# EmbersArc/EiCOS

Measured on NVIDIA B200. Metric: SOCP solves/sec, higher is better.
Workload: dtype f64

## Files before the change

### eicos_b200/csrc/engine.cu

```cuda
#include "engine.hpp"
#include "backend.hpp"
#include "tile_program.hpp"

#include <algorithm>
#include <cstdint>
#ifdef EICOS_EMU
#include <thread>
#endif

namespace eicos
{

#ifndef EICOS_EMU
#define EI_DEFINE_KERNEL(name, fn, minblocks) EI_DEFINE_KERNEL_(name, fn, EI_MAX_THREADS, minblocks, 0)
#define EI_DEFINE_KERNEL1(name, fn) EI_DEFINE_KERNEL_(name, fn, 32, 8, 0)
#define EI_DEFINE_KERNEL_(name, fn, maxthreads, minblocks, JOBS)                                           \
    __global__ void __launch_bounds__(maxthreads, minblocks) name(const __grid_constant__ KArgs a) \
    {                                                                                          \
        extern __shared__ double smem[];                                                       \
        Team tm;                                                                               \
        tm.pl = threadIdx.x & 31;                                                              \
        tm.lane = tm.pl * VEC;                                                                 \
        tm.wk = threadIdx.x >> 5;                                                              \
        tm.nwk = blockDim.x >> 5;                                                              \
// ... 58 lines not shown
                fn(tm_, (args), tile_);                                                           \
            };                                                                                    \
            std::vector<std::thread> th_;                                                         \
            for (int wk_ = 1; wk_ < nw_; wk_++)                                                   \
                th_.emplace_back(body_, wk_);                                                     \
            body_(0);                                                                             \
            for (auto &t_ : th_)                                                                  \
                t_.join();                                                                        \
        }                                                                                         \
    } while (0)
#endif

#ifdef EICOS_EMU
static void eicos_compact_emu(const KArgs &a, const MoveRanges &mr, const int *moves, int nmoves)
{
    for (int q = 0; q < nmoves; q++)
    {
        compact_move(a, mr, moves[2 * q], moves[2 * q + 1], 0, 1);
        compact_vacate(a, moves[2 * q]);
    }
}
#endif

constexpr int MAX_SW_SLOTS = 16, MAX_FA_SLOTS = 24;

int Engine::tile_width() { return TILE; }

bool Engine::pair_solves(int) const { return force_pair_ > 0; }

bool Engine::deep_ring(int ctas) const
{
    if (force_variant_ >= 0)
        return force_variant_ > 0;
    long long per_sm = (long long)((size_t)227 * 1024 / (smem_prog_[M_VARIANTS - 1] + 1024));
    if (const char *v = std::getenv("EICOS_DEEP_CTAS_PER_SM"))
        per_sm = std::atoi(v);
    return (long long)ctas <= per_sm * sms_;
}

bool Engine::wide_launch(int ctas) const
{
    if (force_wide_ >= 0)
        return force_wide_ > 0;
    const long long per_sm = (long long)((size_t)227 * 1024 / (smem_wide_ + 1024));
    return per_sm > 0 && (long long)ctas <= per_sm * sms_;
}

namespace
{
template <class T>
T *upload(const std::vector<T> &v, std::vector<void *> &owned, be::stream_t s)
{
    T *d = (T *)be::alloc(v.size() * sizeof(T));
    be::h2d(d, v.data(), v.size() * sizeof(T), s);
    owned.push_back(d);
    return d;
}
inline be::stream_t S_(void *p) { return (be::stream_t)(intptr_t)p; }

dvec expanded_geq(const Symbolic &S)
{
    dvec g(S.mt, 1.0);
    for (int i = 0; i < S.m; i++)
        g[S.zk[i]] = S.Geq[i];
    return g;
}
}

void Engine::build_layout(const Symbolic &S, bool acc_rows)
{
    int at = 0;
    auto take = [&](int rows) {
        const int o = at;
        at += rows;
        return o;
    };
    Layout &L = L_;
    L.chb = take(S.N);
    L.w = take(S.N);
    L.s = take(S.mt);
    L.lam = take(S.mt);
    L.wb = take(S.N);
    L.bs = take(S.mt);
    L.blam = take(S.mt);
    L.r = take(S.N);
    L.lpv = take(S.l);
    L.lpw = take(S.l);
    L.cpar = take(S.nc * CP_COUNT);
    L.cq = take(S.qtot);
    L.V = take((int)S.Vslot.size());
    L.Lx = take(S.nnzL);
    L.D = take(S.N);
    L.Dinv = take(S.N);
    L.rhs1 = take(S.N);
    L.rhs2 = take(S.N);
    L.sol1 = take(S.N);
    L.sol2 = take(S.N);
    L.xw = take(S.N);
    L.dxr = take(S.N);
    L.e = take(S.N);
    L.xw2 = take(S.N);
    L.dxr2 = take(S.N);
    L.e2 = take(S.N);
    L.dsw = take(S.mt);
    L.wdz = take(S.mt);
    L.dsaff = take(S.mt);
    L.ds1 = take(S.mt);
    L.Gx = take(pim_ ? S.G.nnz() : 0);
    L.Ax = take(pim_ ? S.A.nnz() : 0);
    L.eq = take(pim_ ? S.N : 0);
    L.sc = take(S_COUNT);
    L.acc = acc_rows ? take(S.nnzL) : -1;
    L.rows_total = at;
    L.irows_total = J_COUNT;
}

void Engine::upload_pattern(const Symbolic &S)
{
    be::stream_t st = S_(stream_);
    int sw_budget = MAX_SW_SLOTS, fa_budget = MAX_FA_SLOTS;
    if (const char *v = std::getenv("EICOS_MAX_SW_SLOTS"))
        sw_budget = std::max(1, std::min(MAX_SW_SLOTS, std::atoi(v)));
    if (const char *v = std::getenv("EICOS_MAX_FA_SLOTS"))
        fa_budget = std::max(1, std::min(MAX_FA_SLOTS, std::atoi(v)));
    try
    {
        build_streams(S, L_, workers_, sw_budget, fa_budget, H_, pim_);
    }
    catch (const MachineOutOfSlots &)
    {
        if (L_.acc >= 0)
            throw;
        build_layout(S, true);
        build_streams(S, L_, workers_, sw_budget, fa_budget, H_, pim_);
    }
    Lp_ = S.Lp;
    DevPattern &P = P_;
    P.n = S.n;
    P.p = S.p;
    P.m = S.m;
    P.l = S.l;
    P.nc = S.nc;
    P.N = S.N;
    P.mt = S.mt;
    P.qtot = S.qtot;
    P.nnzL = S.nnzL;
    P.nnzV = (int)S.Vslot.size();
    P.maxcol = S.maxcol;
    P.pim = pim_ ? 1 : 0;
    P.nnzG = S.G.nnz();
    P.nnzA = S.A.nnz();
    if (pim_)
    {
        P.Gp = upload(S.G.p, owned_, st);
        P.Gi = upload(S.G.i, owned_, st);
        P.Ap = upload(S.A.p, owned_, st);
        P.Ai = upload(S.A.i, owned_, st);
        P.Grp = upload(S.Gr.p, owned_, st);
        P.Grv = upload(S.Gr.v, owned_, st);
        P.Arp = upload(S.Ar.p, owned_, st);
        P.Arv = upload(S.Ar.v, owned_, st);
        P.cone_z = upload(S.cone_z, owned_, st);
    }
    P.cone_dim = upload(S.q, owned_, st);
    P.cone_k = upload(S.cone_k, owned_, st);
    P.cone_q = upload(S.cone_q, owned_, st);
    P.zk = upload(S.zk, owned_, st);
// ... 410 lines not shown
            a.initialize = init;
            pick(2 * tiles);
            if (pair_solves(tiles))
            {
                a.njobs = 1;
                EI_TIMED(1, EI_LAUNCH(eicos_solve_kkt_pair, tile_solve_kkt<2>, tiles, threads1, smem_pair_, st, a));
            }
            else if (wide_launch(2 * tiles))
            {
                a.variant = force_variant_ == 0 ? 0 : M_VARIANTS - 1;
                EI_TIMED(1, EI_LAUNCH_JOBS(eicos_solve_kkt_wide, tile_solve_kkt<1>, tiles, 2, threads_wide, smem_wide_, st, a));
            }
            else
                EI_TIMED(1, EI_LAUNCH_JOBS(eicos_solve_kkt, tile_solve_kkt<1>, tiles, 2, threads1, smem_prog_[a.variant], st, a));
            stt.solve_launches++;
            stt.solve_launch_tiles += (long long)tiles * 2;
        };
        auto kkt_rhs2 = [&](int nitrow) {
            a.job[0] = {L_.rhs2, L_.sol2, nitrow, 1};
            a.njobs = 1;
            a.initialize = 0;
            pick(tiles);
            if (wide_launch(tiles))
            {
                a.variant = force_variant_ == 0 ? 0 : M_VARIANTS - 1;
                EI_TIMED(1, EI_LAUNCH_JOBS(eicos_solve_kkt_wide, tile_solve_kkt<1>, tiles, 1, threads_wide, smem_wide_, st, a));
            }
            else
                EI_TIMED(1, EI_LAUNCH_JOBS(eicos_solve_kkt, tile_solve_kkt<1>, tiles, 1, threads1, smem_prog_[a.variant], st, a));
            stt.solve_launches++;
            stt.solve_launch_tiles += tiles;
        };

        EI_TIMED(2, EI_LAUNCH(eicos_load_inputs, tile_load, tiles, threads, smem_common_, st, a));
        if (pim_)
            EI_TIMED(2, EI_LAUNCH(eicos_equilibrate, tile_equil, tiles, threads, smem_common_, st, a));
        EI_TIMED(2, EI_LAUNCH(eicos_init, tile_init, tiles, threads, smem_common_, st, a));
        factor();
        kkt_pair(1, J_NIT1, J_NIT2);
        EI_TIMED(2, EI_LAUNCH(eicos_init_point, tile_init_point, tiles, threads, smem_common_, st, a));

        for (int it = 0; it <= iter_max_ + 1; it++)
        {
            be::zero(active_count_, sizeof(unsigned int), st);
            if (wide_launch(tiles))
                EI_TIMED(3, EI_LAUNCH(eicos_residuals_wide, tile_resid, tiles, threads_wide, smem_wide_, st, a));
            else
                EI_TIMED(3, EI_LAUNCH(eicos_residuals, tile_resid, tiles, threads1, smem_resid_, st, a));
            EI_TIMED(4, EI_LAUNCH(eicos_iter_head, tile_head, tiles, threads, smem_common_, st, a));
            stt.resid_launches++, stt.vector_launches++;
            stt.resid_launch_tiles += tiles, stt.vector_launch_tiles += tiles;
            stt.ipm_iterations++;
            be::d2h(host_pinned_, active_count_, sizeof(unsigned int), st);
            be::sync(st);
            const long long nactive = host_pinned_[0];
            if (nactive == 0)
                break;
            if (compaction_ && !keep_sticky && tiles >= 8 && nactive * 4 <= (long long)tiles * TILE * 3)
            {
                EI_TIMED(2, EI_LAUNCH(eicos_store_outputs, tile_store, tiles, threads, smem_common_, st, a));
                be::d2h_2d(status_host_, TILE * sizeof(int), iws_ + (size_t)J_STATUS * TILE,
                           (size_t)L_.irows_total * TILE * sizeof(int), TILE * sizeof(int), tiles, st);
                be::sync(st);
                const int new_tiles = (int)((nactive + TILE - 1) / TILE);
                int nmoves = 0, hole = 0;
                const int keep = new_tiles * TILE;
                for (int src = keep; src < tiles * TILE; src++)
                {
                    if (status_host_[src] != ST_ACTIVE)
                        continue;
                    while (hole < keep && status_host_[hole] == ST_ACTIVE)
                        hole++;
                    if (hole >= keep)
                        throw std::logic_error("compaction: no free slot");
                    moves_host_[2 * nmoves] = src;
                    moves_host_[2 * nmoves + 1] = hole++;
                    nmoves++;
                }
                if (nmoves > 0)
                {
                    be::h2d(moves_dev_, moves_host_, 2 * (size_t)nmoves * sizeof(int), st);
                    MoveRanges mr;
                    const int rr[14] = {L_.chb, P_.N,
                                        L_.w, (L_.blam + P_.mt) - L_.w,
                                        L_.r, P_.N,
                                        L_.lpv, (L_.V + P_.nnzV) - L_.lpv,
                                        L_.rhs1, 2 * P_.N,
                                        L_.sc, S_COUNT,
                                        L_.Gx, L_.sc - L_.Gx};
                    mr.n = 7;
                    for (int k = 0; k < 14; k++)
                        mr.r[k] = rr[k];
#ifndef EICOS_EMU
                    eicos_compact<<<nmoves, 128, 0, st>>>(a, mr, moves_dev_);
#else
                    eicos_compact_emu(a, mr, moves_dev_, nmoves);
#endif
                    stt.launches++;
                    stt.compactions++;
                }
                tiles = new_tiles;
            }
            factor();
            kkt_pair(0, -1, -1);
            EI_TIMED(4, EI_LAUNCH(eicos_iter_mid, tile_mid, tiles, threads, smem_common_, st, a));
            kkt_rhs2(J_NIT3);
            EI_TIMED(4, EI_LAUNCH(eicos_iter_tail, tile_tail, tiles, threads, smem_common_, st, a));
            stt.vector_launches += 2;
            stt.vector_launch_tiles += 2 * (long long)tiles;
        }
        EI_TIMED(2, EI_LAUNCH(eicos_store_outputs, tile_store, tiles, threads, smem_common_, st, a));
    }
    be::d2h(host_pinned_ + 2, ir_rounds_, 8 * sizeof(unsigned long long), st);
#ifndef EICOS_EMU
    if (timing)
    {
        ev_end = ev();
        EI_CUDA(cudaEventRecord(ev_end, st));
    }
    EI_CUDA(cudaGetLastError());
#endif
    be::sync(st);
    std::memcpy(&stt.ir_rounds, host_pinned_ + 2, sizeof(unsigned long long));
    std::memcpy(&stt.lane_rounds, host_pinned_ + 2 + 2 * 6, sizeof(unsigned long long));
    std::memcpy(stt.kkt_phase_cycles, host_pinned_ + 4, 5 * sizeof(unsigned long long));
#ifndef EICOS_EMU
    if (timing)
    {
        float ms = 0;
        EI_CUDA(cudaEventElapsedTime(&ms, ev_begin, ev_end));
        stt.ms_total = ms;
        for (const Span &sp : spans)
        {
            EI_CUDA(cudaEventElapsedTime(&ms, sp.a, sp.b));
            (sp.cls == 0 ? stt.ms_factor : sp.cls == 1 ? stt.ms_solve : stt.ms_other) += ms;
            if (sp.cls == 3)
                stt.ms_resid += ms;
            if (sp.cls == 4)
                stt.ms_vector += ms;
        }
    }
#endif
#undef EI_TIMED
}

void Engine::debug_factor_init(int batch, const double *d_c, const double *d_h, const double *d_b,
                               const double *base_c, const double *base_h, const double *base_b,
                               double *h_Lx, double *h_D, double *h_sol1, double *h_sol2, int *h_nit)
{
    be::set_device(device_);
    be::stream_t st = S_(stream_);
    if (batch > cap_tiles_ * TILE)
        throw std::invalid_argument("debug_factor_init: batch exceeds workspace capacity");
    KArgs a;
    std::memset(&a, 0, sizeof(a));
    a.P = P_;
    a.L = L_;
    a.ws = ws_;
    a.iws = iws_;
    a.in_c = d_c;
    a.in_h = d_h;
    a.in_b = d_b;
    a.base_c = base_vec_;
    a.base_h = base_vec_ + P_.n;
    a.base_b = base_vec_ + P_.n + P_.m;
    if (base_c)
        be::h2d(base_vec_, base_c, P_.n * sizeof(double), st);
// ... 70 lines not shown
```

### eicos_b200/csrc/layout.hpp

```cpp
#pragma once

#include <cstddef>

namespace eicos
{

enum : int
{
    ST_ACTIVE = -1000,
    EXIT_OPTIMAL = 0,
    EXIT_PINF = 1,
    EXIT_DINF = 2,
    EXIT_MAXIT = -1,
    EXIT_NUMERICS = -2,
    EXIT_OUTCONE = -3,
    EXIT_FATAL = -7,
    EXIT_INACC = 10,
    EXIT_NOT_CONVERGED = -87
};

enum ScalarRow : int
{
    S_KAP, S_TAU, S_CX, S_BY, S_HZ,
    S_PCOST, S_DCOST, S_PRES, S_DRES, S_PINFRES, S_DINFRES, S_GAP, S_RELGAP,
    S_SIGMA, S_MU, S_STEP, S_STEP_AFF, S_KAPOVERT,
    S_WORK_END,
    S_BEST = S_WORK_END,
    S_BEST_END = S_BEST + S_WORK_END,
    S_RT = S_BEST_END, S_NX, S_NY, S_NZ, S_NS, S_HRESX, S_HRESY, S_HRESZ,
    S_RESX0, S_RESY0, S_RESZ0, S_PRES_PREV,
    S_DTAU_DENOM, S_DTAUAFF, S_DKAPAFF,
    S_RHSMAX1, S_RHSMAX2,
    S_RED,
    S_COUNT = S_RED + 14
};

enum IntRow : int
{
    J_ITER, J_PINF, J_DINF, J_HAS_PINFRES, J_HAS_DINFRES, J_HAS_RELGAP, J_NIT1, J_NIT2, J_NIT3,
    J_WORK_END,
    J_BEST = J_WORK_END,
    J_BEST_END = J_BEST + J_WORK_END,
    J_STATUS = J_BEST_END,
    J_INST,
    J_STORED,
    J_COUNT
};

struct Layout
{
    int chb;
    int w;
    int s, lam;
    int wb, bs, blam;
    int r;
    int lpv, lpw;
    int cpar, cq;
    int V;
    int Lx, D, Dinv;
    int rhs1, rhs2, sol1, sol2;
    int xw, dxr, e;
    int xw2, dxr2, e2;
    int dsw, wdz, dsaff, ds1;
    int Gx, Ax, eq;
    int sc;
    int acc;
    int rows_total;
    int irows_total;
};

struct DevMachine
{
    const int *ops;
    int nchunks;
    int nld_chunks;
    int ring_groups;
    int ring_row0;
};

enum ConeParam : int
{
    CP_ETA, CP_ETA2, CP_A, CP_D1, CP_U0, CP_U1, CP_V1, CP_W, CP_COUNT
};

struct DevPattern
{
    int n, p, m, l, nc, N, mt, qtot, nnzL, nnzV, maxcol;
    const int *cone_dim, *cone_k, *cone_q;
    const int *zk;
    const double *xeq, *Aeq, *GeqE;
    DevMachine fw[2], bw[2], bwp[2], mv[2];
    const int *fw_ld[2][2][2], *bw_ld[2][2][2], *mv_ld[2][2];
    DevMachine rs[4], mvw[4];
    const int *rs_ld[4], *mvw_ld[2][4];
    DevMachine fw2, bw2, bwp2, mv2;
    const int *fw2_ld[2], *bw2_ld[2], *mv2_ld;
    int mv_rows;
    int sw_budget, fa_budget, pair_budget;
    DevMachine fa[2];
    const int *fa_ld[2];
    int pim, nnzG, nnzA;
    const int *Gp, *Gi, *Ap, *Ai, *Grp, *Grv, *Arp, *Arv, *cone_z;
    const int *Vkind;
};

}
```

### eicos_b200/csrc/tile_program.hpp

```cpp
#pragma once

#include "layout.hpp"
#include "streams.hpp"
#include "symbolic.hpp"

#include <cfloat>
#include <cmath>

#ifdef EICOS_EMU
#include <barrier>
#define EI_DEV inline
#define EI_LDG(p) (*(p))
#define EI_CLOCK() 0ll
#else
#include <cuda_runtime.h>
#define EI_DEV __device__ __forceinline__
#define EI_LDG(p) __ldg(p)
#define EI_CLOCK() clock64()
#endif

#ifndef EICOS_VEC
#define EICOS_VEC 2
#endif

namespace eicos
{

#ifdef EICOS_EMU
constexpr int LANES = 1;
#else
constexpr int LANES = 32;
#endif
constexpr int VEC = EICOS_VEC;
constexpr int TILE = LANES * VEC;
constexpr int KRED = 7;

struct alignas(VEC >= 2 ? 16 : 8) vd
{
    double v[VEC];
};
struct vb
{
    bool v[VEC];
};
#define VFOR for (int c_ = 0; c_ < VEC; c_++)

EI_DEV vd vset(double s)
{
    vd r;
    VFOR r.v[c_] = s;
    return r;
}
EI_DEV vd operator+(vd a, vd b) { VFOR a.v[c_] += b.v[c_]; return a; }
EI_DEV vd operator-(vd a, vd b) { VFOR a.v[c_] -= b.v[c_]; return a; }
EI_DEV vd operator*(vd a, vd b) { VFOR a.v[c_] *= b.v[c_]; return a; }
EI_DEV vd operator/(vd a, vd b) { VFOR a.v[c_] /= b.v[c_]; return a; }
EI_DEV vd operator-(vd a) { VFOR a.v[c_] = -a.v[c_]; return a; }
EI_DEV vd operator+(vd a, double b) { VFOR a.v[c_] += b; return a; }
EI_DEV vd operator-(vd a, double b) { VFOR a.v[c_] -= b; return a; }
EI_DEV vd operator+(double b, vd a) { VFOR a.v[c_] = b + a.v[c_]; return a; }
EI_DEV vd operator-(double b, vd a) { VFOR a.v[c_] = b - a.v[c_]; return a; }
EI_DEV vd operator*(vd a, double b) { VFOR a.v[c_] *= b; return a; }
EI_DEV vd operator*(double b, vd a) { VFOR a.v[c_] = b * a.v[c_]; return a; }
EI_DEV vd operator/(vd a, double b) { VFOR a.v[c_] /= b; return a; }
EI_DEV vd operator/(double b, vd a) { VFOR a.v[c_] = b / a.v[c_]; return a; }
EI_DEV vd &operator+=(vd &a, vd b) { VFOR a.v[c_] += b.v[c_]; return a; }
EI_DEV vd &operator-=(vd &a, vd b) { VFOR a.v[c_] -= b.v[c_]; return a; }
EI_DEV vd vfnma(vd v, vd a, vd b)
{
    VFOR v.v[c_] = fma(-a.v[c_], b.v[c_], v.v[c_]);
    return v;
}
EI_DEV vd vfnma(vd v, double a, vd b)
{
    VFOR v.v[c_] = fma(-a, b.v[c_], v.v[c_]);
    return v;
}
EI_DEV vd vsqrt(vd a) { VFOR a.v[c_] = sqrt(a.v[c_]); return a; }
EI_DEV vd vabs(vd a) { VFOR a.v[c_] = fabs(a.v[c_]); return a; }
EI_DEV bool ei_isnan(double v) { return v != v; }
EI_DEV double dmax(double a, double b) { return a > b ? a : b; }
EI_DEV double dmin(double a, double b) { return b < a ? b : a; }
EI_DEV vd vmax(vd a, vd b) { VFOR a.v[c_] = dmax(a.v[c_], b.v[c_]); return a; }
EI_DEV vd vmin(vd a, vd b) { VFOR a.v[c_] = dmin(a.v[c_], b.v[c_]); return a; }
EI_DEV vd vsel(vb m, vd a, vd b) { VFOR a.v[c_] = m.v[c_] ? a.v[c_] : b.v[c_]; return a; }
EI_DEV vb vbset(bool s)
{
    vb r;
    VFOR r.v[c_] = s;
    return r;
}
EI_DEV vb operator&&(vb a, vb b) { VFOR a.v[c_] = a.v[c_] && b.v[c_]; return a; }
EI_DEV vb operator||(vb a, vb b) { VFOR a.v[c_] = a.v[c_] || b.v[c_]; return a; }
EI_DEV vb operator!(vb a) { VFOR a.v[c_] = !a.v[c_]; return a; }
EI_DEV bool vany(vb a)
{
    bool r = false;
    VFOR r = r || a.v[c_];
    return r;
}
EI_DEV bool vall(vb a)
{
    bool r = true;
    VFOR r = r && a.v[c_];
    return r;
}

EI_DEV vd vload(const double *p) { return *reinterpret_cast<const vd *>(p); }
EI_DEV void vstore(double *p, vd v) { *reinterpret_cast<vd *>(p) = v; }

#ifdef EICOS_EMU
struct i4
{
    int x, y, z, w;
};
EI_DEV i4 ldg4(const int *p) { return i4{p[0], p[1], p[2], p[3]}; }
#else
typedef int4 i4;
EI_DEV i4 ldg4(const int *p) { return __ldg(reinterpret_cast<const int4 *>(p)); }
#endif
struct alignas(16) d2
{
    double x, y;
};
EI_DEV d2 ldg2(const double *p)
{
#ifdef EICOS_EMU
    return d2{p[0], p[1]};
#else
    const double2 v = __ldg(reinterpret_cast<const double2 *>(p));
    return d2{v.x, v.y};
#endif
}

struct RowRef
{
    double *p;
    EI_DEV operator vd() const { return vload(p); }
    EI_DEV void operator=(vd v) const { vstore(p, v); }
    EI_DEV void operator=(double s) const { vstore(p, vset(s)); }
    EI_DEV void operator+=(vd v) const { vstore(p, vload(p) + v); }
    EI_DEV void operator-=(vd v) const { vstore(p, vload(p) - v); }
    EI_DEV void operator*=(double s) const { vstore(p, vload(p) * s); }
    EI_DEV void operator*=(vd s) const { vstore(p, vload(p) * s); }
    EI_DEV void operator=(const RowRef &o) const { vstore(p, vload(o.p)); }
};
#define ROWD(base, r) (RowRef{(base) + (size_t)(r) * TILE})
#define ROWC(base, r, c) ((base)[(size_t)(r) * TILE + (c)])

struct KArgs
{
    DevPattern P;
    Layout L;
    double *ws;
    int *iws;
    int batch;
    int first;
    const double *in_c, *in_h, *in_b;
    const double *base_c, *base_h, *base_b;
// ... 1440 lines not shown
        const vd res = resv[0], b = bv[0], own = ownv[0];
        if (kind == RS_PRE_X)
            r[RS_HX2] += res * res;
        else if (kind == RS_PRE_Y)
            r[RS_HY2] += res * res;
        else if (kind == RS_PRE_Z)
            r[RS_HZ2] += res * res;
        else
        {
            if (kind == RS_FIN_X)
            {
                r[RS_RX2] += res * res;
                r[RS_CX] += b * own;
                r[RS_NX2] += own * own;
            }
            else if (kind == RS_FIN_Y)
            {
                r[RS_RY2] += res * res;
                r[RS_BY] += b * own;
                r[RS_NY2] += own * own;
            }
            else if (kind == RS_FIN_Z)
            {
                r[RS_RZ2] += res * res;
                r[RS_HZ] += b * own;
                r[RS_NZ2] += own * own;
            }
            else
            {
                r[RS_NS2] += res * res;
                r[RS_GAP] += res * own;
                if (kind == RS_FIRST_PRE_Z)
                    r[RS_HZ2] += res * res;
            }
        }
    }
};

EI_DEV void tile_resid(const Team &tm, const KArgs &a, int tile)
{
    const TileMem t = tile_mem(tm, a, tile);
    const vb act = lane_active(tm, t);
    if (!tm.any(act))
        return;
    const DevPattern &P = a.P;
    const Layout &L = a.L;
    double *T = t.T;
    const bool wide = tm.nwk >= M_MV_PARTS;
    vd tot[RS_NRED];
    for (int k = 0; k < RS_NRED; k++)
        tot[k] = vset(0.0);
    const auto run_part = [&](int part, double *mem) {
        ResidFin fin;
        for (int k = 0; k < RS_NRED; k++)
            fin.r[k] = vset(0.0);
        Machine mm;
        mm.init(tm, mem);
        MRun r;
        r.prog = P.rs[part];
        r.ld = P.rs_ld[part];
        r.Tb = t.Tb;
        r.out = r.out2 = r.outB = r.out2B = T + (size_t)L.r * TILE;
        r.a_one = false;
        mm.run<MC_CONST | MC_POS | MC_BKEEP | MC_FIN | MC_X3, 1>(tm, r, fin);
        for (int k = 0; k < RS_NRED; k++)
            tot[k] = part == 0 || wide ? fin.r[k] : tot[k] + fin.r[k];
    };
    if (P.mv_rows > 0)
    {
        if (wide)
        {
            if (tm.wk < M_MV_PARTS)
                run_part(tm.wk, tm.pbuf + (size_t)tm.wk * a.part_doubles);
            team_sum<RS_NRED>(tm, tot);
        }
        else if (tm.wk == 0)
            for (int part = 0; part < M_MV_PARTS; part++)
                run_part(part, tm.pbuf);
    }
    if (tm.wk == 0)
        for (int k = 0; k < RS_NRED; k++)
            ROWD(T, L.sc + S_RED + k) = tot[k];
}

EI_DEV void tile_head(const Team &tm, const KArgs &a, int tile)
{
    const TileMem t = tile_mem(tm, a, tile);
    const vb act = lane_active(tm, t);
    if (!tm.any(act))
        return;
    const DevPattern &P = a.P;
    const Layout &L = a.L;
    double *T = t.T;
    int *I = t.I;
    const int n = P.n, p = P.p, zb = P.n + P.p;
    const vd tau = ROWD(T, L.sc + S_TAU), kap = ROWD(T, L.sc + S_KAP);
    enum { HX2, RX2, CX, NX2, HY2, RY2, BY, NY2, HZ2, RZ2, HZ, NZ2, NS2, GAP, NRED };
    static_assert(NRED == 14, "S_RED holds 14 rows");
    vd r[NRED];
    for (int k = 0; k < NRED; k++)
        r[k] = ROWD(T, L.sc + S_RED + k);

    vb restore = vbset(false), save = vbset(false), fin = vbset(false), cont = vbset(false);
    vd ftau = tau;
    WState wsv[VEC], bsv[VEC];
    double rtv[VEC], ppv[VEC];
    int codev[VEC];
    VFOR
    {
        const int c = c_;
        WState &w = wsv[c], &best = bsv[c];
        ws_load(tm, T, I, L.sc, 0, 0, c, w);
        ws_load(tm, T, I, L.sc, S_BEST, J_BEST, c, best);
        const double tau_c = tau.v[c], kap_c = kap.v[c];
        const double hresx = sqrt(r[HX2].v[c]), hresy = sqrt(r[HY2].v[c]), hresz = sqrt(r[HZ2].v[c]);
        const double nx = sqrt(r[NX2].v[c]), ny = sqrt(r[NY2].v[c]), nz = sqrt(r[NZ2].v[c]), ns = sqrt(r[NS2].v[c]);
        const double cx = r[CX].v[c], by = p > 0 ? r[BY].v[c] : 0., hz = r[HZ].v[c];
        const double rt = kap_c + cx + by + hz;
        w.d[S_CX] = cx;
        w.d[S_BY] = by;
        w.d[S_HZ] = hz;
        w.d[S_GAP] = r[GAP].v[c];
        w.d[S_MU] = (r[GAP].v[c] + kap_c * tau_c) / ((P.l + P.nc) + 1);
        w.d[S_KAPOVERT] = kap_c / tau_c;
        w.d[S_PCOST] = cx / tau_c;
        w.d[S_DCOST] = -(hz + by) / tau_c;
        if (w.d[S_PCOST] < 0.)
        {
            w.i[J_HAS_RELGAP] = 1;
            w.d[S_RELGAP] = w.d[S_GAP] / (-w.d[S_PCOST]);
        }
        else if (w.d[S_DCOST] > 0.)
        {
            w.i[J_HAS_RELGAP] = 1;
            w.d[S_RELGAP] = w.d[S_GAP] / w.d[S_DCOST];
        }
        else
            w.i[J_HAS_RELGAP] = 0;
        const double resx0 = ROWC(T, L.sc + S_RESX0, c), resy0 = ROWC(T, L.sc + S_RESY0, c), resz0 = ROWC(T, L.sc + S_RESZ0, c);
        const double nry = p > 0 ? sqrt(r[RY2].v[c]) / dmax(resy0 + nx, 1.) : 0.;
        const double nrz = sqrt(r[RZ2].v[c]) / dmax(resz0 + nx + ns, 1.);
        w.d[S_PRES] = dmax(nry, nrz) / tau_c;
        w.d[S_DRES] = sqrt(r[RX2].v[c]) / dmax(resx0 + ny + nz, 1.) / tau_c;
        if ((hz + by) / dmax(ny + nz, 1.) < -Settings::reltol)
        {
            w.i[J_HAS_PINFRES] = 1;
            w.d[S_PINFRES] = hresx / dmax(ny + nz, 1.);
        }
        if (cx / dmax(nx, 1.) < -Settings::reltol)
        {
            w.i[J_HAS_DINFRES] = 1;
            w.d[S_DINFRES] = dmax(hresy / dmax(nx, 1.), hresz / dmax(nx + ns, 1.));
        }

        const int iter = w.i[J_ITER];
        double pres_prev = ROWC(T, L.sc + S_PRES_PREV, c);
        int code = ST_ACTIVE;
        bool rst = false, sav = false;
        if (act.v[c])
        {
            if (iter > 0 && (w.d[S_PRES] > Settings::safeguard * pres_prev || w.d[S_GAP] < 0.))
            {
                rst = true;
                w = best;
                code = ws_check_exit(w, true);
                if (code == EXIT_NOT_CONVERGED)
                    code = EXIT_NUMERICS;
            }
            else
            {
                pres_prev = w.d[S_PRES];
                code = ws_check_exit(w, false);
                if (code == EXIT_NOT_CONVERGED)
                {
                    if (iter > 0 && w.d[S_STEP] == Settings::stepmin * Settings::gamma)
                    {
                        rst = true;
                        w = best;
                        code = ws_check_exit(w, true);
                        if (code == EXIT_NOT_CONVERGED)
                            code = EXIT_NUMERICS;
                    }
                    else if (iter == a.iter_max)
                    {
                        if (!ws_better(w, best))
                        {
                            rst = true;
                            w = best;
                        }
                        code = ws_check_exit(w, true);
                        if (code == EXIT_NOT_CONVERGED)
                            code = EXIT_MAXIT;
                    }
                    else if (ei_isnan(w.d[S_PCOST]))
                    {
                        if (!(iter == 0 || ws_better(w, best)))
                        {
                            rst = true;
                            w = best;
                            code = ws_check_exit(w, true);
                            if (code == EXIT_NOT_CONVERGED)
                                code = EXIT_NUMERICS;
                        }
                    }
                    else
                        code = ST_ACTIVE;
                }
            }
            if (code == ST_ACTIVE && (iter == 0 || ws_better(w, best)))
            {
                sav = true;
                best = w;
            }
        }
        restore.v[c] = rst;
        save.v[c] = sav;
        fin.v[c] = act.v[c] && code != ST_ACTIVE;
        cont.v[c] = act.v[c] && code == ST_ACTIVE;
        ftau.v[c] = w.d[S_TAU];
        rtv[c] = rt;
        ppv[c] = pres_prev;
        codev[c] = code;
    }
    tm.sync();
    if (tm.wk == 0)
        VFOR if (act.v[c_])
        {
            ws_store(tm, T, I, L.sc, 0, 0, c_, wsv[c_]);
            if (save.v[c_])
                ws_store(tm, T, I, L.sc, S_BEST, J_BEST, c_, bsv[c_]);
            ROWC(T, L.sc + S_RT, c_) = rtv[c_];
            ROWC(T, L.sc + S_PRES_PREV, c_) = ppv[c_];
            ROWC(I, J_STATUS, c_) = codev[c_];
        }

    if (!tm.any(restore || fin) && tm.all(save || !act))
    {
        const int ins[1] = {L.w};
        ew_rows<1, 8>(tm, T, P.N, ins, [&](int q, const vd *x) { ROWD(T, L.wb + q) = x[0]; });
        const int inz[2] = {L.s, L.lam};
        ew_rows<2, 6>(tm, T, P.mt, inz, [&](int e, const vd *x) {
            ROWD(T, L.bs + e) = x[0];
            ROWD(T, L.blam + e) = x[1];
        });
    }
    else if (tm.any(restore || save || fin))
    {
        const bool any_fin = tm.any(fin);
        {
            const int ins[2] = {L.w, L.wb};
            ew_rows<2, 6>(tm, T, P.N, ins, [&](int q, const vd *x) {
                vd v = vsel(restore, x[1], x[0]);
                ROWD(T, L.wb + q) = vsel(save, v, x[1]);
                if (any_fin && P.pim)
                    v = vsel(fin, v / (vd(ROWD(T, L.eq + q)) * ftau), v);
                else if (any_fin)
                {
                    const double eq = q < n ? EI_LDG(P.xeq + q) : (q < zb ? EI_LDG(P.Aeq + q - n) : EI_LDG(P.GeqE + q - zb));
                    v = vsel(fin, v / (eq * ftau), v);
                }
                ROWD(T, L.w + q) = v;
            });
        }
        {
            const int ins[4] = {L.s, L.lam, L.bs, L.blam};
            ew_rows<4, 3>(tm, T, P.mt, ins, [&](int e, const vd *x) {
                vd sv = vsel(restore, x[2], x[0]), lv = vsel(restore, x[3], x[1]);
                ROWD(T, L.bs + e) = vsel(save, sv, x[2]);
                ROWD(T, L.blam + e) = vsel(save, lv, x[3]);
                if (any_fin && P.pim)
                    sv = vsel(fin, sv * (vd(ROWD(T, L.eq + zb + e)) / ftau), sv);
                else if (any_fin)
                    sv = vsel(fin, sv * (EI_LDG(P.GeqE + e) / ftau), sv);
                ROWD(T, L.s + e) = sv;
                ROWD(T, L.lam + e) = lv;
            });
        }
    }
    if (!tm.any(cont))
        return;
    tm.sync();
#ifndef EICOS_EMU
    if (tm.wk == 0 && a.active_count)
    {
        int mine = 0;
        VFOR mine += cont.v[c_] ? 1 : 0;
        for (int o = 16; o > 0; o >>= 1)
            mine += __shfl_xor_sync(0xffffffffu, mine, o);
        if (tm.pl == 0)
            atomicAdd(a.active_count, (unsigned)mine);
    }
#else
    if (tm.wk == 0 && a.active_count)
        VFOR if (cont.v[c_]) *a.active_count += 1;
#endif

    const int sz = L.w + zb;
    const bool lp_only = P.nc == 0;
    if (lp_only && tm.all(cont))
    {
        const int ins[2] = {L.s, sz};
        ew_rows<2, 6>(tm, T, P.l, ins, [&](int k, const vd *x) {
            const vd v = x[0] / x[1];
            const vd w = vsqrt(v);
            ROWD(T, L.lpv + k) = -v;
            ROWD(T, L.lpw + k) = w;
            ROWD(T, L.V + k) = -v - Settings::deltastat;
            ROWD(T, L.lam + k) = w * x[1];
        });
    }
    else if (lp_only)
    {
        const int ins[5] = {L.s, sz, L.lpv, L.lpw, L.lam};
        ew_rows<5, 2>(tm, T, P.l, ins, [&](int k, const vd *x) {
            const vd v = x[0] / x[1];
            const vd nvn = vsel(cont, -v, x[2]);
            const vd wn = vsel(cont, vsqrt(v), x[3]);
            ROWD(T, L.lpv + k) = nvn;
            ROWD(T, L.lpw + k) = wn;
            ROWD(T, L.V + k) = nvn - Settings::deltastat;
            ROWD(T, L.lam + k) = vsel(cont, wn * x[1], x[4]);
        });
    }
    else
    {
        const int ins[4] = {L.s, sz, L.lpv, L.lpw};
        ew_rows<4, 3>(tm, T, P.l, ins, [&](int k, const vd *x) {
            const vd v = x[0] / x[1];
            const vd nvn = vsel(cont, -v, x[2]);
            ROWD(T, L.lpv + k) = nvn;
            ROWD(T, L.lpw + k) = vsel(cont, vsqrt(v), x[3]);
            ROWD(T, L.V + k) = nvn - Settings::deltastat;
        });
    }
    vb nofail = vbset(true);
    if (P.nc > 0)
    {
        vd ff[1] = {vset((double)P.nc)};
        for (int c = tm.wk; c < P.nc; c += tm.nwk)
        {
            const int ks = EI_LDG(P.cone_k + c), d = EI_LDG(P.cone_dim + c);
            VFOR
            {
                const ConeScaling cs = cone_scaling(tm, T, L.s + ks, sz + ks, d, c_);
                if (cs.stage != 0)
                    ff[0].v[c_] = dmin(ff[0].v[c_], (double)c);
            }
        }
        team_min<1>(tm, ff);
        VFOR nofail.v[c_] = (int)ff[0].v[c_] == P.nc;
        for (int c = tm.wk; c < P.nc; c += tm.nwk)
        {
            const int d = EI_LDG(P.cone_dim + c), ks = EI_LDG(P.cone_k + c), qo = EI_LDG(P.cone_q + c);
            const int cp = L.cpar + c * CP_COUNT;
            VFOR
            {
                if (!cont.v[c_] || c > (int)ff[0].v[c_])
                    continue;
                const ConeScaling cs = cone_scaling(tm, T, L.s + ks, sz + ks, d, c_);
                if (cs.stage == 1)
                    continue;
                ROWC(T, cp + CP_ETA2, c_) = cs.eta2;
                ROWC(T, cp + CP_ETA, c_) = cs.eta;
                for (int k = 1; k < d; k++)
                    ROWC(T, L.cq + qo + k - 1, c_) = (0.5 / cs.gamma) * (ROWC(T, L.s + ks + k, c_) / cs.snorm - ROWC(T, sz + ks + k, c_) / cs.znorm);
                if (cs.stage == 2)
                    continue;
                ROWC(T, cp + CP_D1, c_) = cs.d1;
                ROWC(T, cp + CP_U0, c_) = cs.u0;
                ROWC(T, cp + CP_U1, c_) = cs.u1;
                ROWC(T, cp + CP_V1, c_) = cs.v1;
                ROWC(T, cp + CP_A, c_) = cs.a;
                ROWC(T, cp + CP_W, c_) = cs.w;
            }
        }
    }
    tm.sync();
    if (!lp_only)
        cone_scale(tm, a, T, sz, L.lam, cont && nofail);

    const double delta = Settings::deltastat;
    for (int c = tm.wk; c < P.nc; c += tm.nwk)
    {
        const int d = EI_LDG(P.cone_dim + c), ks = EI_LDG(P.cone_k + c), qo = EI_LDG(P.cone_q + c);
        const int cp = L.cpar + c * CP_COUNT;
        const vd eta2 = ROWD(T, cp + CP_ETA2), d1 = ROWD(T, cp + CP_D1), u0 = ROWD(T, cp + CP_U0);
        const vd u1 = ROWD(T, cp + CP_U1), v1 = ROWD(T, cp + CP_V1);
        int vb_ = L.V + P.l + 3 * (ks - 2 * c - P.l) + c;
        ROWD(T, vb_++) = -(eta2 * d1) - delta;
        for (int k = 1; k < d; k++)
            ROWD(T, vb_++) = -eta2 - delta;
        ROWD(T, vb_++) = -eta2;
        for (int k = 1; k < d; k++)
            ROWD(T, vb_++) = -(eta2 * v1) * vd(ROWD(T, L.cq + qo + k - 1));
        ROWD(T, vb_++) = eta2 + delta;
        ROWD(T, vb_++) = -(eta2 * u0);
        for (int k = 1; k < d; k++)
            ROWD(T, vb_++) = -(eta2 * u1) * vd(ROWD(T, L.cq + qo + k - 1));
    }
    {
        vd mx[1] = {vset(0.0)};
        const int ins[1] = {L.r};
        ew_rows<1, 8>(tm, T, zb, ins, [&](int q, const vd *x) {
            ROWD(T, L.rhs2 + q) = q < n ? x[0] : -x[0];
            mx[0] = vmax(mx[0], vabs(x[0]));
        });
        const int inz[2] = {L.s, L.r + zb};
        ew_rows<2, 6>(tm, T, P.mt, inz, [&](int e, const vd *x) {
            const vd v = x[0] - x[1];
            ROWD(T, L.rhs2 + zb + e) = v;
            mx[0] = vmax(mx[0], vabs(v));
        });
        team_max<1>(tm, mx);
        if (tm.wk == 0)
            ROWD(T, L.sc + S_RHSMAX2) = vsel(cont, mx[0], ROWD(T, L.sc + S_RHSMAX2));
    }
}

EI_DEV void tile_mid(const Team &tm, const KArgs &a, int tile)
{
    const TileMem t = tile_mem(tm, a, tile);
    const vb act = lane_active(tm, t);
    if (!tm.any(act))
        return;
    const DevPattern &P = a.P;
    const Layout &L = a.L;
    double *T = t.T;
    const int n = P.n, p = P.p, zb = P.n + P.p;
    const vd tau = ROWD(T, L.sc + S_TAU), kap = ROWD(T, L.sc + S_KAP), rt = ROWD(T, L.sc + S_RT);
    const vd mu = ROWD(T, L.sc + S_MU);

    vd dt[6];
    for (int k = 0; k < 6; k++)
        dt[k] = vset(0.0);
    {
        const int ix[3] = {L.chb, L.sol1, L.sol2};
        ew_rows<3, 4>(tm, T, n, ix, [&](int, const vd *x) {
            dt[0] += x[0] * x[1];
            dt[3] += x[0] * x[2];
        });
        const int iy[3] = {L.chb + n, L.sol1 + n, L.sol2 + n};
        ew_rows<3, 4>(tm, T, p, iy, [&](int, const vd *x) {
            dt[1] += x[0] * x[1];
            dt[4] += x[0] * x[2];
        });
        const int iz[3] = {L.chb + zb, L.sol1 + zb, L.sol2 + zb};
        ew_rows<3, 4>(tm, T, P.l, iz, [&](int, const vd *x) {
            dt[2] += x[0] * x[1];
            dt[5] += x[0] * x[2];
        });
    }
    for (int c = tm.wk; c < P.nc; c += tm.nwk)
    {
        const int d = EI_LDG(P.cone_dim + c), kb = zb + EI_LDG(P.cone_k + c);
        for (int k = 0; k < d; k++)
        {
            const vd hv = ROWD(T, L.chb + kb + k);
            dt[2] += hv * vd(ROWD(T, L.sol1 + kb + k));
            dt[5] += hv * vd(ROWD(T, L.sol2 + kb + k));
        }
    }
    team_sum<6>(tm, dt);
    const vd dtau_denom = kap / tau - dt[0] - dt[1] - dt[2];
    const vd dtauaff = (rt - kap + dt[3] + dt[4] + dt[5]) / dtau_denom;
    vd m0 = vset(DBL_MAX), m1 = vset(DBL_MAX);
    {
        const int ins[4] = {L.sol2 + zb, L.sol1 + zb, L.lpw, L.lam};
        ew_rows<4, 3>(tm, T, P.l, ins, [&](int k, const vd *x) {
            const vd dz = x[0] + dtauaff * x[1];
            const vd wd = x[2] * dz;
            const vd ds = -wd - x[3];
            ROWD(T, L.sol2 + zb + k) = dz;
            ROWD(T, L.wdz + k) = wd;
            ROWD(T, L.dsw + k) = ds;
            m0 = vmin(m0, ds / x[3]);
            m1 = vmin(m1, wd / x[3]);
        });
    }
    if (P.mt > P.l)
    {
        const int cz = zb + P.l, nr = P.mt - P.l;
        const int ins[2] = {L.sol2 + cz, L.sol1 + cz};
        ew_rows<2, 6>(tm, T, nr, ins, [&](int e, const vd *x) { ROWD(T, L.sol2 + cz + e) = x[0] + dtauaff * x[1]; });
        tm.sync();
        cone_scale(tm, a, T, L.sol2 + zb, L.wdz, vbset(true), false);
        tm.sync();
        const int in2[2] = {L.wdz + P.l, L.lam + P.l};
        ew_rows<2, 6>(tm, T, nr, in2, [&](int e, const vd *x) { ROWD(T, L.dsw + P.l + e) = -x[0] - x[1]; });
        tm.sync();
    }
    const vd dkapaff = -kap - kap / tau * dtauaff;
    const vd step_aff = line_search(tm, a, T, L.lam, L.dsw, L.wdz, tau, dtauaff, kap, dkapaff, false, m0, m1);
    vd sigma;
    VFOR
    {
        const double om = 1. - step_aff.v[c_];
        double sg = om * om * om;
        if (sg < Settings::sigmamin)
            sg = Settings::sigmamin;
        else if (Settings::sigmamax < sg)
            sg = Settings::sigmamax;
        sigma.v[c_] = sg;
    }
    if (tm.wk == 0)
        VFOR if (act.v[c_])
        {
            ROWC(T, L.sc + S_DTAU_DENOM, c_) = dtau_denom.v[c_];
            ROWC(T, L.sc + S_DTAUAFF, c_) = dtauaff.v[c_];
            ROWC(T, L.sc + S_DKAPAFF, c_) = dkapaff.v[c_];
            ROWC(T, L.sc + S_STEP_AFF, c_) = step_aff.v[c_];
            ROWC(T, L.sc + S_SIGMA, c_) = sigma.v[c_];
        }

    const vd sigmamu = sigma * mu, oms = 1. - sigma;
    vd mx[1] = {vset(0.0)};
    {
        const int ins[1] = {L.rhs2};
        ew_rows<1, 8>(tm, T, n + p, ins, [&](int r, const vd *x) {
            const vd v = x[0] * oms;
            ROWD(T, L.rhs2 + r) = v;
            mx[0] = vmax(mx[0], vabs(v));
        });
        const int inl[5] = {L.lam, L.dsw, L.wdz, L.r + zb, L.lpw};
        ew_rows<5, 2>(tm, T, P.l, inl, [&](int k, const vd *x) {
            const vd lk = x[0];
            vd d1 = lk * lk;
            d1 += x[1] * x[2];
            d1 -= sigmamu;
            const vd q = d1 / lk;
            ROWD(T, L.dsw + k) = q;
            const vd v = -oms * x[3] + x[4] * q;
            ROWD(T, L.rhs2 + zb + k) = v;
            mx[0] = vmax(mx[0], vabs(v));
        });
    }
    for (int c = tm.wk; c < P.nc; c += tm.nwk)
    {
        const int d = EI_LDG(P.cone_dim + c), zs = EI_LDG(P.cone_k + c), qo = EI_LDG(P.cone_q + c);
        const int kb = zb + zs;
        const int cp = L.cpar + c * CP_COUNT;
        const vd eta = ROWD(T, cp + CP_ETA), ca = ROWD(T, cp + CP_A);
        const vd l0 = ROWD(T, L.lam + zs), u0 = ROWD(T, L.dsw + zs), v0 = ROWD(T, L.wdz + zs);
        vd ll = vset(0.0), uv = vset(0.0);
        for (int k = 0; k < d; k++)
        {
            const vd lk = ROWD(T, L.lam + zs + k);
            ll += lk * lk;
            uv += vd(ROWD(T, L.dsw + zs + k)) * vd(ROWD(T, L.wdz + zs + k));
        }
        vd w0 = ll - sigmamu;
        w0 += uv;
        ROWD(T, L.ds1 + zs) = w0;
        for (int k = 1; k < d; k++)
        {
            const vd lk = ROWD(T, L.lam + zs + k);
            vd v = l0 * lk + l0 * lk;
            v += u0 * vd(ROWD(T, L.wdz + zs + k)) + v0 * vd(ROWD(T, L.dsw + zs + k));
            ROWD(T, L.ds1 + zs + k) = v;
        }
        vd rho = vset(0.0), zeta = vset(0.0);
        for (int k = 1; k < d; k++)
        {
            const vd lk = ROWD(T, L.lam + zs + k);
            rho += lk * lk;
            zeta += lk * vd(ROWD(T, L.ds1 + zs + k));
        }
        rho = l0 * l0 - rho;
        const vd factor = (zeta / l0 - w0) / rho;
        const vd q0 = (l0 * w0 - zeta) / rho;
        ROWD(T, L.dsw + zs) = q0;
        for (int k = 1; k < d; k++)
            ROWD(T, L.dsw + zs + k) = factor * vd(ROWD(T, L.lam + zs + k)) + vd(ROWD(T, L.ds1 + zs + k)) / l0;
        vd zt = vset(0.0);
        for (int k = 1; k < d; k++)
            zt += vd(ROWD(T, L.cq + qo + k - 1)) * vd(ROWD(T, L.dsw + zs + k));
        const vd fz = q0 + zt / (1. + ca);
        {
            const vd v = -oms * vd(ROWD(T, L.r + kb)) + eta * (ca * q0 + zt);
            ROWD(T, L.rhs2 + kb) = v;
            mx[0] = vmax(mx[0], vabs(v));
        }
        for (int k = 1; k < d; k++)
        {
            const vd v = -oms * vd(ROWD(T, L.r + kb + k)) +
                         eta * (vd(ROWD(T, L.dsw + zs + k)) + fz * vd(ROWD(T, L.cq + qo + k - 1)));
            ROWD(T, L.rhs2 + kb + k) = v;
            mx[0] = vmax(mx[0], vabs(v));
        }
        ROWD(T, L.rhs2 + kb + d) = 0.0;
        ROWD(T, L.rhs2 + kb + d + 1) = 0.0;
    }
    team_max<1>(tm, mx);
    if (tm.wk == 0)
        ROWD(T, L.sc + S_RHSMAX2) = vsel(act, mx[0], ROWD(T, L.sc + S_RHSMAX2));
}

EI_DEV void tile_tail(const Team &tm, const KArgs &a, int tile)
{
    const TileMem t = tile_mem(tm, a, tile);
    const vb act = lane_active(tm, t);
    if (!tm.any(act))
        return;
    const DevPattern &P = a.P;
    const Layout &L = a.L;
    double *T = t.T;
    const int n = P.n, zb = P.n + P.p;
    const vd tau = ROWD(T, L.sc + S_TAU), kap = ROWD(T, L.sc + S_KAP), rt = ROWD(T, L.sc + S_RT);
    const vd mu = ROWD(T, L.sc + S_MU), sigma = ROWD(T, L.sc + S_SIGMA);
    const vd dtau_denom = ROWD(T, L.sc + S_DTAU_DENOM), dtauaff = ROWD(T, L.sc + S_DTAUAFF);
    const vd dkapaff = ROWD(T, L.sc + S_DKAPAFF);

    vd dt[3] = {vset(0.0), vset(0.0), vset(0.0)};
    {
        const int ix[2] = {L.chb, L.sol2};
        ew_rows<2, 6>(tm, T, n, ix, [&](int, const vd *x) { dt[0] += x[0] * x[1]; });
        const int iy[2] = {L.chb + n, L.sol2 + n};
        ew_rows<2, 6>(tm, T, P.p, iy, [&](int, const vd *x) { dt[1] += x[0] * x[1]; });
        const int iz[2] = {L.chb + zb, L.sol2 + zb};
        ew_rows<2, 6>(tm, T, P.l, iz, [&](int, const vd *x) { dt[2] += x[0] * x[1]; });
    }
    for (int c = tm.wk; c < P.nc; c += tm.nwk)
    {
        const int d = EI_LDG(P.cone_dim + c), kb = zb + EI_LDG(P.cone_k + c);
        for (int k = 0; k < d; k++)
            dt[2] += vd(ROWD(T, L.chb + kb + k)) * vd(ROWD(T, L.sol2 + kb + k));
    }
    team_sum<3>(tm, dt);
    const vd bkap = kap * tau + dkapaff * dtauaff - sigma * mu;
    const vd dtau = ((1. - sigma) * rt - bkap / tau + dt[0] + dt[1] + dt[2]) / dtau_denom;
    {
        const int ins[2] = {L.sol2, L.sol1};
        ew_rows<2, 6>(tm, T, zb, ins, [&](int r, const vd *x) { ROWD(T, L.sol2 + r) = x[0] + dtau * x[1]; });
    }
    vd m0 = vset(DBL_MAX), m1 = vset(DBL_MAX);
    {
        const int ins[5] = {L.sol2 + zb, L.sol1 + zb, L.lpw, L.dsw, L.lam};
        ew_rows<5, 2>(tm, T, P.l, ins, [&](int k, const vd *x) {
            const vd dz = x[0] + dtau * x[1];
            const vd wd = x[2] * dz;
            const vd ds = -(x[3] + wd);
            ROWD(T, L.sol2 + zb + k) = dz;
            ROWD(T, L.dsw + k) = ds;
            m0 = vmin(m0, ds / x[4]);
            m1 = vmin(m1, wd / x[4]);
        });
    }
    if (P.mt > P.l)
    {
        const int cz = zb + P.l, nr = P.mt - P.l;
        const int ins[2] = {L.sol2 + cz, L.sol1 + cz};
        ew_rows<2, 6>(tm, T, nr, ins, [&](int e, const vd *x) { ROWD(T, L.sol2 + cz + e) = x[0] + dtau * x[1]; });
        tm.sync();
        cone_scale(tm, a, T, L.sol2 + zb, L.wdz, vbset(true), false);
        tm.sync();
        const int in2[2] = {L.dsw + P.l, L.wdz + P.l};
        ew_rows<2, 6>(tm, T, nr, in2, [&](int e, const vd *x) { ROWD(T, L.dsw + P.l + e) = -(x[0] + x[1]); });
        tm.sync();
    }
    const vd dkap = -(bkap + kap * dtau) / tau;
    const vd step = Settings::gamma * line_search(tm, a, T, L.lam, L.dsw, L.wdz, tau, dtau, kap, dkap, false, m0, m1);
    if (P.mt > P.l)
    {
        cone_scale(tm, a, T, L.dsw, L.dsaff, vbset(true), false);
        tm.sync();
    }
    {
        const int ins[2] = {L.w, L.sol2};
        ew_rows<2, 6>(tm, T, zb, ins, [&](int q, const vd *x) { ROWD(T, L.w + q) = vsel(act, x[0] + step * x[1], x[0]); });
        const int inl[5] = {L.w + zb, L.sol2 + zb, L.s, L.lpw, L.dsw};
        ew_rows<5, 2>(tm, T, P.l, inl, [&](int k, const vd *x) {
            ROWD(T, L.w + zb + k) = vsel(act, x[0] + step * x[1], x[0]);
            ROWD(T, L.s + k) = vsel(act, x[2] + step * (x[3] * x[4]), x[2]);
        });
    }
    for (int c = tm.wk; c < P.nc; c += tm.nwk)
    {
        const int d = EI_LDG(P.cone_dim + c), kb = zb + EI_LDG(P.cone_k + c);
        for (int k = 0; k < d; k++)
            ROWD(T, L.w + kb + k) = vsel(act, vd(ROWD(T, L.w + kb + k)) + step * vd(ROWD(T, L.sol2 + kb + k)), ROWD(T, L.w + kb + k));
    }
    if (P.mt > P.l)
    {
        const int ins[2] = {L.s + P.l, L.dsaff + P.l};
        ew_rows<2, 6>(tm, T, P.mt - P.l, ins, [&](int e, const vd *x) { ROWD(T, L.s + P.l + e) = vsel(act, x[0] + step * x[1], x[0]); });
    }
    if (tm.wk == 0)
        VFOR if (act.v[c_])
        {
            ROWC(T, L.sc + S_KAP, c_) = kap.v[c_] + step.v[c_] * dkap.v[c_];
            ROWC(T, L.sc + S_TAU, c_) = tau.v[c_] + step.v[c_] * dtau.v[c_];
            ROWC(T, L.sc + S_STEP, c_) = step.v[c_];
            ROWC(t.I, J_ITER, c_) += 1;
        }
}

EI_DEV void tile_load(const Team &tm, const KArgs &a, int tile)
{
    const TileMem t = tile_mem(tm, a, tile);
    const DevPattern &P = a.P;
    const Layout &L = a.L;
    const int n = P.n, zb = P.n + P.p;
    VFOR
    {
        int inst = tile * TILE + tm.lane + c_;
        if (inst >= a.batch)
            inst = a.batch - 1;
        const size_t g = (size_t)a.first + inst;
        if (P.pim)
        {
            for (int j = tm.wk; j < n; j += tm.nwk)
                ROWC(t.T, L.chb + j, c_) = a.in_c ? a.in_c[g * n + j] : EI_LDG(a.base_c + j);
            for (int i = tm.wk; i < P.p; i += tm.nwk)
                ROWC(t.T, L.chb + n + i, c_) = a.in_b ? a.in_b[g * P.p + i] : EI_LDG(a.base_b + i);
            for (int i = tm.wk; i < P.m; i += tm.nwk)
                ROWC(t.T, L.chb + zb + EI_LDG(P.zk + i), c_) = a.in_h ? a.in_h[g * P.m + i] : EI_LDG(a.base_h + i);
            for (int k = tm.wk; k < P.nnzG; k += tm.nwk)
                ROWC(t.T, L.Gx + k, c_) = a.in_G ? a.in_G[g * P.nnzG + k] : EI_LDG(a.base_G + k);
            for (int k = tm.wk; k < P.nnzA; k += tm.nwk)
                ROWC(t.T, L.Ax + k, c_) = a.in_A ? a.in_A[g * P.nnzA + k] : EI_LDG(a.base_A + k);
            continue;
        }
        for (int j = tm.wk; j < n; j += tm.nwk)
        {
            const double v = a.in_c ? a.in_c[g * n + j] : EI_LDG(a.base_c + j);
            ROWC(t.T, L.chb + j, c_) = a.pre_equilibrated ? v : v / EI_LDG(P.xeq + j);
        }
        for (int i = tm.wk; i < P.p; i += tm.nwk)
        {
            const double v = a.in_b ? a.in_b[g * P.p + i] : EI_LDG(a.base_b + i);
            ROWC(t.T, L.chb + n + i, c_) = a.pre_equilibrated ? v : v / EI_LDG(P.Aeq + i);
        }
        for (int i = tm.wk; i < P.m; i += tm.nwk)
        {
            const double v = a.in_h ? a.in_h[g * P.m + i] : EI_LDG(a.base_h + i);
            const int e = EI_LDG(P.zk + i);
            ROWC(t.T, L.chb + zb + e, c_) = a.pre_equilibrated ? v : v / EI_LDG(P.GeqE + e);
        }
    }
}

template <class RowOf>
EI_DEV vd equil_max_abs(const double *T, int k0, int k1, vd mx, RowOf row)
{
    int k = k0;
    for (; k + 4 <= k1; k += 4)
    {
        vd v[4];
#pragma unroll
        for (int u = 0; u < 4; u++)
            v[u] = vload(T + (size_t)row(k + u) * TILE);
#pragma unroll
        for (int u = 0; u < 4; u++)
            mx = vmax(vabs(v[u]), mx);
    }
    for (; k < k1; k++)
// ... 189 lines not shown
```

Before: 44360.

## Recompute LP lambda and search directions on the fly instead of storing rows

Drops the stored backup lambda row and, for pure-LP problems, derives lambda as lpw times z instead of keeping it in memory. The affine and combined steps now recompute dz, wd and ds from sol1/sol2 inside the consuming loops rather than writing and re-reading intermediate rows, which cuts global memory traffic per iteration. It uses explicit fma and __dmul_rn to keep results reproducible. The cost is some redundant arithmetic, slightly different rounding, and a smaller compaction footprint tied to the new layout.

```diff
diff --git a/eicos_b200/csrc/engine.cu b/eicos_b200/csrc/engine.cu
--- a/eicos_b200/csrc/engine.cu
+++ b/eicos_b200/csrc/engine.cu
@@ -164,7 +164,6 @@
     L.lam = take(S.mt);
     L.wb = take(S.N);
     L.bs = take(S.mt);
-    L.blam = take(S.mt);
     L.r = take(S.N);
     L.lpv = take(S.l);
     L.lpw = take(S.l);
@@ -741,7 +740,7 @@
                     be::h2d(moves_dev_, moves_host_, 2 * (size_t)nmoves * sizeof(int), st);
                     MoveRanges mr;
                     const int rr[14] = {L_.chb, P_.N,
-                                        L_.w, (L_.blam + P_.mt) - L_.w,
+                                        L_.w, (L_.bs + P_.mt) - L_.w,
                                         L_.r, P_.N,
                                         L_.lpv, (L_.V + P_.nnzV) - L_.lpv,
                                         L_.rhs1, 2 * P_.N,
diff --git a/eicos_b200/csrc/layout.hpp b/eicos_b200/csrc/layout.hpp
--- a/eicos_b200/csrc/layout.hpp
+++ b/eicos_b200/csrc/layout.hpp
@@ -52,7 +52,7 @@
     int chb;
     int w;
     int s, lam;
-    int wb, bs, blam;
+    int wb, bs;
     int r;
     int lpv, lpw;
     int cpar, cq;
diff --git a/eicos_b200/csrc/tile_program.hpp b/eicos_b200/csrc/tile_program.hpp
--- a/eicos_b200/csrc/tile_program.hpp
+++ b/eicos_b200/csrc/tile_program.hpp
@@ -75,6 +75,24 @@
 {
     VFOR v.v[c_] = fma(-a, b.v[c_], v.v[c_]);
     return v;
+}
+EI_DEV vd vfma(vd a, vd b, vd c)
+{
+    VFOR c.v[c_] = fma(a.v[c_], b.v[c_], c.v[c_]);
+    return c;
+}
+EI_DEV vd vmul_rn(vd a, vd b)
+{
+#ifdef EICOS_EMU
+    VFOR
+    {
+        a.v[c_] *= b.v[c_];
+        asm("" : "+x"(a.v[c_]));
+    }
+#else
+    VFOR a.v[c_] = __dmul_rn(a.v[c_], b.v[c_]);
+#endif
+    return a;
 }
 EI_DEV vd vsqrt(vd a) { VFOR a.v[c_] = sqrt(a.v[c_]); return a; }
 EI_DEV vd vabs(vd a) { VFOR a.v[c_] = fabs(a.v[c_]); return a; }
@@ -1681,6 +1699,9 @@
         for (int k = 0; k < RS_NRED; k++)
             ROWD(T, L.sc + S_RED + k) = tot[k];
 }
+
+EI_DEV int lp_lambda_row(const DevPattern &P, const Layout &L) { return P.nc == 0 ? L.w + P.n + P.p : L.lam; }
+EI_DEV vd lp_lambda(const DevPattern &P, vd lpw, vd row) { return P.nc == 0 ? vmul_rn(lpw, row) : row; }
 
 EI_DEV void tile_head(const Team &tm, const KArgs &a, int tile)
 {
@@ -1837,11 +1858,8 @@
     {
         const int ins[1] = {L.w};
         ew_rows<1, 8>(tm, T, P.N, ins, [&](int q, const vd *x) { ROWD(T, L.wb + q) = x[0]; });
-        const int inz[2] = {L.s, L.lam};
-        ew_rows<2, 6>(tm, T, P.mt, inz, [&](int e, const vd *x) {
-            ROWD(T, L.bs + e) = x[0];
-            ROWD(T, L.blam + e) = x[1];
-        });
+        const int inz[1] = {L.s};
+        ew_rows<1, 8>(tm, T, P.mt, inz, [&](int e, const vd *x) { ROWD(T, L.bs + e) = x[0]; });
     }
     else if (tm.any(restore || save || fin))
     {
@@ -1862,17 +1880,15 @@
             });
         }
         {
-            const int ins[4] = {L.s, L.lam, L.bs, L.blam};
-            ew_rows<4, 3>(tm, T, P.mt, ins, [&](int e, const vd *x) {
-                vd sv = vsel(restore, x[2], x[0]), lv = vsel(restore, x[3], x[1]);
-                ROWD(T, L.bs + e) = vsel(save, sv, x[2]);
-                ROWD(T, L.blam + e) = vsel(save, lv, x[3]);
+            const int ins[2] = {L.s, L.bs};
+            ew_rows<2, 6>(tm, T, P.mt, ins, [&](int e, const vd *x) {
+                vd sv = vsel(restore, x[1], x[0]);
+                ROWD(T, L.bs + e) = vsel(save, sv, x[1]);
                 if (any_fin && P.pim)
                     sv = vsel(fin, sv * (vd(ROWD(T, L.eq + zb + e)) / ftau), sv);
                 else if (any_fin)
                     sv = vsel(fin, sv * (EI_LDG(P.GeqE + e) / ftau), sv);
                 ROWD(T, L.s + e) = sv;
-                ROWD(T, L.lam + e) = lv;
             });
         }
     }
@@ -1901,24 +1917,9 @@
         const int ins[2] = {L.s, sz};
         ew_rows<2, 6>(tm, T, P.l, ins, [&](int k, const vd *x) {
             const vd v = x[0] / x[1];
-            const vd w = vsqrt(v);
             ROWD(T, L.lpv + k) = -v;
-            ROWD(T, L.lpw + k) = w;
+            ROWD(T, L.lpw + k) = vsqrt(v);
             ROWD(T, L.V + k) = -v - Settings::deltastat;
-            ROWD(T, L.lam + k) = w * x[1];
-        });
-    }
-    else if (lp_only)
-    {
-        const int ins[5] = {L.s, sz, L.lpv, L.lpw, L.lam};
-        ew_rows<5, 2>(tm, T, P.l, ins, [&](int k, const vd *x) {
-            const vd v = x[0] / x[1];
-            const vd nvn = vsel(cont, -v, x[2]);
-            const vd wn = vsel(cont, vsqrt(v), x[3]);
-            ROWD(T, L.lpv + k) = nvn;
-            ROWD(T, L.lpw + k) = wn;
-            ROWD(T, L.V + k) = nvn - Settings::deltastat;
-            ROWD(T, L.lam + k) = vsel(cont, wn * x[1], x[4]);
         });
     }
     else
@@ -2062,18 +2063,16 @@
     team_sum<6>(tm, dt);
     const vd dtau_denom = kap / tau - dt[0] - dt[1] - dt[2];
     const vd dtauaff = (rt - kap + dt[3] + dt[4] + dt[5]) / dtau_denom;
+    const int lrow = lp_lambda_row(P, L);
     vd m0 = vset(DBL_MAX), m1 = vset(DBL_MAX);
     {
-        const int ins[4] = {L.sol2 + zb, L.sol1 + zb, L.lpw, L.lam};
-        ew_rows<4, 3>(tm, T, P.l, ins, [&](int k, const vd *x) {
-            const vd dz = x[0] + dtauaff * x[1];
-            const vd wd = x[2] * dz;
-            const vd ds = -wd - x[3];
-            ROWD(T, L.sol2 + zb + k) = dz;
-            ROWD(T, L.wdz + k) = wd;
-            ROWD(T, L.dsw + k) = ds;
-            m0 = vmin(m0, ds / x[3]);
-            m1 = vmin(m1, wd / x[3]);
+        const int ins[4] = {L.sol2 + zb, L.sol1 + zb, L.lpw, lrow};
+        ew_rows<4, 3>(tm, T, P.l, ins, [&](int, const vd *x) {
+            const vd lk = lp_lambda(P, x[2], x[3]);
+            const vd wd = vmul_rn(x[2], vfma(dtauaff, x[1], x[0]));
+            const vd ds = -wd - lk;
+            m0 = vmin(m0, ds / lk);
+            m1 = vmin(m1, wd / lk);
         });
     }
     if (P.mt > P.l)
@@ -2120,11 +2119,13 @@
             ROWD(T, L.rhs2 + r) = v;
             mx[0] = vmax(mx[0], vabs(v));
         });
-        const int inl[5] = {L.lam, L.dsw, L.wdz, L.r + zb, L.lpw};
+        const int inl[5] = {lrow, L.sol2 + zb, L.sol1 + zb, L.r + zb, L.lpw};
         ew_rows<5, 2>(tm, T, P.l, inl, [&](int k, const vd *x) {
-            const vd lk = x[0];
+            const vd lk = lp_lambda(P, x[4], x[0]);
+            const vd wd = vmul_rn(x[4], vfma(dtauaff, x[2], x[1]));
+            const vd ds = -wd - lk;
             vd d1 = lk * lk;
-            d1 += x[1] * x[2];
+            d1 += ds * wd;
             d1 -= sigmamu;
             const vd q = d1 / lk;
             ROWD(T, L.dsw + k) = q;
@@ -2227,21 +2228,15 @@
     team_sum<3>(tm, dt);
     const vd bkap = kap * tau + dkapaff * dtauaff - sigma * mu;
     const vd dtau = ((1. - sigma) * rt - bkap / tau + dt[0] + dt[1] + dt[2]) / dtau_denom;
-    {
-        const int ins[2] = {L.sol2, L.sol1};
-        ew_rows<2, 6>(tm, T, zb, ins, [&](int r, const vd *x) { ROWD(T, L.sol2 + r) = x[0] + dtau * x[1]; });
-    }
     vd m0 = vset(DBL_MAX), m1 = vset(DBL_MAX);
     {
-        const int ins[5] = {L.sol2 + zb, L.sol1 + zb, L.lpw, L.dsw, L.lam};
-        ew_rows<5, 2>(tm, T, P.l, ins, [&](int k, const vd *x) {
-            const vd dz = x[0] + dtau * x[1];
-            const vd wd = x[2] * dz;
+        const int ins[5] = {L.sol2 + zb, L.sol1 + zb, L.lpw, L.dsw, lp_lambda_row(P, L)};
+        ew_rows<5, 2>(tm, T, P.l, ins, [&](int, const vd *x) {
+            const vd lk = lp_lambda(P, x[2], x[4]);
+            const vd wd = vmul_rn(x[2], vfma(dtau, x[1], x[0]));
             const vd ds = -(x[3] + wd);
-            ROWD(T, L.sol2 + zb + k) = dz;
-            ROWD(T, L.dsw + k) = ds;
-            m0 = vmin(m0, ds / x[4]);
-            m1 = vmin(m1, wd / x[4]);
+            m0 = vmin(m0, ds / lk);
+            m1 = vmin(m1, wd / lk);
         });
     }
     if (P.mt > P.l)
@@ -2264,12 +2259,14 @@
         tm.sync();
     }
     {
-        const int ins[2] = {L.w, L.sol2};
-        ew_rows<2, 6>(tm, T, zb, ins, [&](int q, const vd *x) { ROWD(T, L.w + q) = vsel(act, x[0] + step * x[1], x[0]); });
-        const int inl[5] = {L.w + zb, L.sol2 + zb, L.s, L.lpw, L.dsw};
-        ew_rows<5, 2>(tm, T, P.l, inl, [&](int k, const vd *x) {
-            ROWD(T, L.w + zb + k) = vsel(act, x[0] + step * x[1], x[0]);
-            ROWD(T, L.s + k) = vsel(act, x[2] + step * (x[3] * x[4]), x[2]);
+        const int ins[3] = {L.w, L.sol2, L.sol1};
+        ew_rows<3, 4>(tm, T, zb, ins, [&](int q, const vd *x) { ROWD(T, L.w + q) = vsel(act, x[0] + step * (x[1] + dtau * x[2]), x[0]); });
+        const int inl[6] = {L.w + zb, L.sol2 + zb, L.sol1 + zb, L.s, L.lpw, L.dsw};
+        ew_rows<6, 2>(tm, T, P.l, inl, [&](int k, const vd *x) {
+            const vd dz = vfma(dtau, x[2], x[1]);
+            const vd ds = -(x[5] + vmul_rn(x[4], dz));
+            ROWD(T, L.w + zb + k) = vsel(act, vfma(step, dz, x[0]), x[0]);
+            ROWD(T, L.s + k) = vsel(act, vfma(step, vmul_rn(x[4], ds), x[3]), x[3]);
         });
     }
     for (int c = tm.wk; c < P.nc; c += tm.nwk)
```

Measured after the change: 45870, median of 6. 3.4% higher.
